# novifinancial/librabft_simulator

Measured on NVIDIA H100. Metric: simulated consensus rounds/sec (whole box), higher is better.
Workload: dtype int64

## Files before the change

__graft_entry__.py:

```python
import os
import sys

ROOT = os.path.dirname(os.path.abspath(__file__))
if ROOT not in sys.path:
    sys.path.insert(0, ROOT)


def build():
    from librabft_simulator_b200 import _build
    _build.build_product(verbose_ptxas=False)
    _build.build_oracle()
    _build.build_hostcore()
    _build.build_sweep_hostcore()
    _build.build_ct_hostcore()
    _build.build_latency_hostcore()
    _build.build_fault_hostcore()
    _build.build_block_latency_hostcore()
    _build.build_block_threshold_probe()
    import librabft_simulator_b200
    from librabft_simulator_b200 import _lib
    _lib.load()


def smoke():
    import numpy as np
    from librabft_simulator_b200 import BatchSimulator, RandomDelay, Simulator
    from tests.support import Oracle
    contexts = Simulator.new(52, 3, RandomDelay.new(10.0, 4.0), None).loop_until(1000)
    assert [c.num_commits() for c in contexts] == [27, 27, 27]
    assert [c.last_committed_state() for c in contexts] == [11134312813757838303] * 3
    seeds = np.arange(1, 65, dtype=np.uint64)
    res = BatchSimulator(seeds, 4, RandomDelay.new(10.0, 4.0)).loop_until(1000)
    ref = Oracle().run(seeds, 4, 1000)
    assert (res.commit_counts == ref.commit_counts).all()
    assert (res.last_committed_states == ref.last_states).all()
    assert (res.counters[:, :8] == ref.counters[:, :8]).all()
    print("smoke ok: 64x4 instances bit-exact vs oracle; rounds/instance = %.1f" % res.active_rounds.mean())


if __name__ == "__main__":
    build()
    print("build ok")
```

librabft_simulator_b200/_build.py:

```python
import os
import shutil
import subprocess

ROOT = os.path.dirname(os.path.dirname(os.path.abspath(__file__)))
CSRC = os.path.join(ROOT, "librabft_simulator_b200", "csrc")
LIB_PATH = os.environ.get("LBFT_LIB_PATH") or os.path.join(CSRC, "liblbft_b200.so")
ORACLE_DIR = os.path.join(ROOT, "oracle")
ORACLE_PATH = os.path.join(ORACLE_DIR, "liblbft_oracle.so")
HOSTCORE_DIR = os.path.join(ROOT, "tests", "hostcore")
HOSTCORE_PATH = os.path.join(HOSTCORE_DIR, "libhostcore.so")
SWEEP_HOSTCORE_PATH = os.path.join(HOSTCORE_DIR, "libhostcore_sweep.so")
CT_HOSTCORE_PATH = os.path.join(HOSTCORE_DIR, "libhostcore_ct.so")
LATENCY_HOSTCORE_PATH = os.path.join(HOSTCORE_DIR, "libhostcore_latency.so")
FAULT_HOSTCORE_PATH = os.path.join(HOSTCORE_DIR, "libhostcore_fault.so")
BLOCK_LATENCY_HOSTCORE_PATH = os.path.join(HOSTCORE_DIR, "libhostcore_block_latency.so")
GPUPROBE_DIR = os.path.join(ROOT, "tests", "gpuprobe")
BLOCK_THRESHOLD_PROBE_PATH = os.path.join(GPUPROBE_DIR, "libblock_threshold_probe.so")

GENCODE = ["-gencode", "arch=compute_90a,code=sm_90a"]
NVCC_FLAGS = GENCODE + ["-lineinfo", "-O3", "-std=c++17", "-Xcompiler", "-fPIC"]
PRODUCT_UNITS = ["lbft_api.cu", "k_fixed.cu", "k_scan.cu", "k_calendar.cu", "k_heap.cu", "k_wide.cu", "k_sweep_thread.cu",
                 "k_sweep_wide.cu", "k_ct_thread.cu", "k_ct_wide.cu", "k_ct_sweep_thread.cu", "k_ct_sweep_wide.cu"]
PRODUCT_HEADERS = ["kernels.cuh", "sim_core.cuh", "sim_params.h", "host_setup.hpp"]


def _newer(target, sources):
    if not os.path.exists(target):
        return False
    t = os.path.getmtime(target)
    return all(os.path.getmtime(s) <= t for s in sources)


def _run(cmd, cwd):
    proc = subprocess.run(cmd, cwd=cwd, stdout=subprocess.PIPE, stderr=subprocess.STDOUT, text=True)
    if proc.returncode != 0:
        raise RuntimeError("build failed: %s\n%s" % (" ".join(cmd), proc.stdout))
    return proc.stdout


def nvcc_path():
    return shutil.which("nvcc") or "/usr/local/cuda/bin/nvcc"


def build_product(force=False, verbose_ptxas=False, lib_path=None):
    from concurrent.futures import ThreadPoolExecutor
    lib_path = lib_path or LIB_PATH
    headers = [os.path.join(CSRC, f) for f in PRODUCT_HEADERS] + [os.path.join(ROOT, "include", "lbft.h")]
    sources = headers + [os.path.join(CSRC, u) for u in PRODUCT_UNITS]
# ... 87 lines not shown
def build_latency_hostcore(force=False):
    srcs = [os.path.join(HOSTCORE_DIR, f) for f in ("latency_hostcore.cpp", "ct_hostcore.cpp")] + [
        os.path.join(ROOT, "include", "lbft.h")] + [os.path.join(CSRC, f) for f in ("sim_core.cuh", "sim_params.h", "host_setup.hpp")] + [
        os.path.join(ORACLE_DIR, f) for f in ("oracle_capi.cpp", "lbft_oracle.hpp")]
    if not force and _newer(LATENCY_HOSTCORE_PATH, srcs):
        return LATENCY_HOSTCORE_PATH
    _run(["g++", "-O2", "-std=c++17", "-fPIC", "-shared", "-ffp-contract=off", "-Wno-unknown-pragmas", "-DLBFT_CHECK_C1",
          "-o", LATENCY_HOSTCORE_PATH, "latency_hostcore.cpp"], HOSTCORE_DIR)
    return LATENCY_HOSTCORE_PATH


def build_fault_hostcore(force=False):
    srcs = [os.path.join(HOSTCORE_DIR, f) for f in ("fault_hostcore.cpp", "ct_hostcore.cpp")] + [
        os.path.join(ROOT, "include", "lbft.h")] + [os.path.join(CSRC, f) for f in ("sim_core.cuh", "sim_params.h", "host_setup.hpp")] + [
        os.path.join(ORACLE_DIR, f) for f in ("oracle_capi.cpp", "lbft_oracle.hpp")]
    if not force and _newer(FAULT_HOSTCORE_PATH, srcs):
        return FAULT_HOSTCORE_PATH
    _run(["g++", "-O2", "-std=c++17", "-fPIC", "-shared", "-ffp-contract=off", "-Wno-unknown-pragmas", "-DLBFT_CHECK_C1",
          "-o", FAULT_HOSTCORE_PATH, "fault_hostcore.cpp"], HOSTCORE_DIR)
    return FAULT_HOSTCORE_PATH


def build_block_latency_hostcore(force=False):
    srcs = [os.path.join(HOSTCORE_DIR, f) for f in ("block_latency_hostcore.cpp", "fault_hostcore.cpp", "ct_hostcore.cpp")] + [
        os.path.join(ROOT, "include", "lbft.h")] + [os.path.join(CSRC, f) for f in ("sim_core.cuh", "sim_params.h", "host_setup.hpp")] + [
        os.path.join(ORACLE_DIR, f) for f in ("oracle_capi.cpp", "lbft_oracle.hpp")]
    if not force and _newer(BLOCK_LATENCY_HOSTCORE_PATH, srcs):
        return BLOCK_LATENCY_HOSTCORE_PATH
    _run(["g++", "-O2", "-std=c++17", "-fPIC", "-shared", "-ffp-contract=off", "-Wno-unknown-pragmas", "-DLBFT_CHECK_C1",
          "-o", BLOCK_LATENCY_HOSTCORE_PATH, "block_latency_hostcore.cpp"], HOSTCORE_DIR)
    return BLOCK_LATENCY_HOSTCORE_PATH


def build_block_threshold_probe(force=False):
    srcs = [os.path.join(GPUPROBE_DIR, "block_threshold_probe.cu")] + [os.path.join(CSRC, f) for f in ("sim_core.cuh", "sim_params.h")]
    if not force and _newer(BLOCK_THRESHOLD_PROBE_PATH, srcs):
        return BLOCK_THRESHOLD_PROBE_PATH
    _run([nvcc_path()] + NVCC_FLAGS + ["-shared", "-o", BLOCK_THRESHOLD_PROBE_PATH, "block_threshold_probe.cu"], GPUPROBE_DIR)
    return BLOCK_THRESHOLD_PROBE_PATH


def build_all(force=False):
    return (build_product(force), build_oracle(force), build_hostcore(force), build_sweep_hostcore(force), build_ct_hostcore(force),
            build_latency_hostcore(force), build_fault_hostcore(force), build_block_latency_hostcore(force),
            build_block_threshold_probe(force))
```

librabft_simulator_b200/csrc/kernels.cuh:

```cuda
#pragma once
#include <cuda_runtime.h>

#include "host_setup.hpp"
#include "sim_core.cuh"

namespace lbft {

LBFT_LAYOUT_FN uint32_t calendar_kmask_words(const Layout& L) { return (L.cal_times + 7) / 8; }

template <int QMODE>
struct LaunchShape {
  static constexpr int kThreads = QMODE == 2 ? 32 * 4 : 32;
  static constexpr int kBlocksPerSm = QMODE == 2 ? 4 : 16;
};

template <int NMAX, int QMODE, int FX, bool REC, bool RES, bool EP, bool TDS, int TILE, bool SW, bool CT = false>
__device__ __forceinline__ void event_loop_body(const Params& P, double* s_zx, double* s_zf, double* s_thr, uint32_t* s_queue,
                                                const uint32_t* set_of, const SweepSet* sets, int32_t* times = nullptr,
                                                bool faults = false) {
  static_assert(TILE == 32 || ((QMODE == 3 || QMODE == 2) && !REC && !RES && !EP && !TDS), "sparse tiles: plain kernels over the calendar / shared-memory queue");
  for (int i = threadIdx.x; i < 257; i += blockDim.x) {
    s_zx[i] = P.zig_x[i];
    s_zf[i] = P.zig_f[i];
  }
  const bool thr_fits = !SW && P.delay_kmax != 0 && P.delay_kmax + 2 <= kThrSmem;
  if (thr_fits)
    for (uint32_t i = threadIdx.x; i < P.delay_kmax + 2; i += blockDim.x) s_thr[i] = P.delay_thr[i];
  __syncthreads();
  const uint32_t gthread = blockIdx.x * blockDim.x + threadIdx.x;
  const uint32_t tile = gthread >> 5, lane = gthread & 31;
  const uint32_t inst = tile * TILE + lane;
  if (lane >= TILE || inst >= P.num_instances) return;
  const uint32_t total_words = FX ? fixed_layout(FX).total_words : P.L.total_words;
  TileMem<TILE> mem{P.state + (size_t)tile * total_words * TILE, lane};
  uint32_t* sk = nullptr;
  uint16_t* sd = nullptr;
  if (QMODE == 2) {
    const uint32_t warp = threadIdx.x >> 5, qcap = P.L.queue_cap;
    uint32_t* base = s_queue + (size_t)warp * (qcap * 32 + qcap * 16);
    sk = base + lane;
    sd = reinterpret_cast<uint16_t*>(base + qcap * 32) + lane;
  }
  constexpr bool KS = QMODE == 3 && TILE < 32;
  Core<TileMem<TILE>, NMAX, QMODE, FX, REC, RES, 1, EP, TDS, KS, SW, CT> core(P, mem, s_zx, s_zf, thr_fits ? s_thr : P.delay_thr, sk, sd);
  if (KS) core.km = s_queue + (size_t)(threadIdx.x >> 5) * calendar_kmask_words(FX ? fixed_layout(FX) : P.L) * TILE + lane;
  if constexpr (CT) core.ct = times + (size_t)inst * (core.L.num_nodes + 1) * core.L.round_cap;
  if constexpr (SW) {
    core.bind_set(faults ? &reinterpret_cast<const SweepSetFaults*>(sets)[set_of[inst]].set : sets + set_of[inst]);
    core.bind_faults(faults);
  }
  if (RES && (P.run_flags & 1u)) core.restore_regs();
  else core.init(P.seeds[inst]);
  core.run();
  core.finalize(inst);
  if (RES) core.save_regs();
}

template <int NMAX, int QMODE, int FX = FX_NONE, bool REC = false, bool RES = false, bool EP = false, bool TDS = false, int TILE = 32>
__global__ void __launch_bounds__(LaunchShape<QMODE>::kThreads, LaunchShape<QMODE>::kBlocksPerSm) lbft_event_loop_kernel(const __grid_constant__ Params P) {
  __shared__ double s_zx[257];
  __shared__ double s_zf[257];
  __shared__ double s_thr[kThrSmem];
  extern __shared__ uint32_t s_queue[];
  event_loop_body<NMAX, QMODE, FX, REC, RES, EP, TDS, TILE, false>(P, s_zx, s_zf, s_thr, s_queue, nullptr, nullptr);
}

template <int NMAX, int QMODE, int TILE = 32>
__global__ void __launch_bounds__(LaunchShape<QMODE>::kThreads, LaunchShape<QMODE>::kBlocksPerSm) lbft_sweep_event_loop_kernel(const __grid_constant__ SweepParams S) {
  __shared__ double s_zx[257];
  __shared__ double s_zf[257];
  extern __shared__ uint32_t s_queue[];
  event_loop_body<NMAX, QMODE, FX_NONE, false, false, false, false, TILE, true>(S.P, s_zx, s_zf, nullptr, s_queue, S.set_of, S.sets, nullptr,
                                                                               S.faults != 0);
}

LBFT_LAYOUT_FN int wide_warps(int g) { return g == 32 ? 1 : 4; }
LBFT_LAYOUT_FN int wide_blocks_per_sm(int g) { return 16 / wide_warps(g); }
// ... 204 lines not shown
```

librabft_simulator_b200/csrc/sim_core.cuh:

```cuda
#pragma once
#include <stddef.h>
#include <stdint.h>

#include <type_traits>

#include "sim_params.h"

#if defined(__CUDACC__)
#define LBFT_HD __host__ __device__ __forceinline__
#define LBFT_COLD inline __host__ __device__ __noinline__
#else
#define LBFT_HD inline
#define LBFT_COLD inline __attribute__((noinline))
#include <cmath>
#endif

namespace lbft {

enum : uint32_t {
  ST_DONE = 1u << 0,
  ST_ROUND_OVERFLOW = 1u << 1,
  ST_QUEUE_OVERFLOW = 1u << 2,
  ST_PAYLOAD_OVERFLOW = 1u << 3,
  ST_INVARIANT = 1u << 4,
// ... 63 lines not shown
  double d;
  __builtin_memcpy(&d, &b, 8);
  return d;
#endif
}
LBFT_HD uint64_t rotl64(uint64_t x, int k) { return (x << k) | (x >> (64 - k)); }
LBFT_HD void st_evict_first(int32_t* p, int32_t v) {
#if defined(__CUDA_ARCH__)
  __stcs(p, v);
#else
  *p = v;
#endif
}

struct SipWords {
  uint64_t v0, v1, v2, v3, nbytes;
  LBFT_HD SipWords() : v0(0x736f6d6570736575ULL), v1(0x646f72616e646f6dULL), v2(0x6c7967656e657261ULL), v3(0x7465646279746573ULL), nbytes(0) {}
  LBFT_HD void round() {
    v0 += v1; v1 = rotl64(v1, 13); v1 ^= v0; v0 = rotl64(v0, 32);
    v2 += v3; v3 = rotl64(v3, 16); v3 ^= v2;
    v0 += v3; v3 = rotl64(v3, 21); v3 ^= v0;
    v2 += v1; v1 = rotl64(v1, 17); v1 ^= v2; v2 = rotl64(v2, 32);
  }
  LBFT_HD void write_u64(uint64_t m) { v3 ^= m; round(); v0 ^= m; nbytes += 8; }
  LBFT_HD uint64_t finish() {
    uint64_t b = nbytes << 56;
    v3 ^= b; round(); v0 ^= b;
    v2 ^= 0xff;
    round(); round(); round();
    return v0 ^ v1 ^ v2 ^ v3;
  }
};

template <int STRIDE_>
struct TileMem {
  static constexpr int STRIDE = STRIDE_;
  uint32_t* tile;
  uint32_t lane;
  LBFT_HD uint32_t* at(uint32_t w) const { return tile + (size_t)w * STRIDE + lane; }
  LBFT_HD uint32_t ld(uint32_t w) const { return tile[(size_t)w * STRIDE + lane]; }
  LBFT_HD void st(uint32_t w, uint32_t v) const { tile[(size_t)w * STRIDE + lane] = v; }
  LBFT_HD uint64_t* at64(uint32_t wbase) const { return reinterpret_cast<uint64_t*>(tile + (size_t)wbase * STRIDE + lane * 2); }
};

template <int NMAX>
struct AuthorList;
template <>
struct AuthorList<16> {
  uint64_t v = 0;
  uint32_t len = 0;
  LBFT_HD void clear() { v = 0; len = 0; }
  LBFT_HD void push(uint32_t a) { v |= (uint64_t)a << (4 * len); len++; }
  LBFT_HD uint32_t get(uint32_t i) const { return (uint32_t)(v >> (4 * i)) & 15u; }
  LBFT_HD void swap(uint32_t i, uint32_t j) {
    uint64_t d = ((v >> (4 * i)) ^ (v >> (4 * j))) & 15u;
    v ^= (d << (4 * i)) | (d << (4 * j));
  }
  LBFT_HD void fill_others(uint32_t n_nodes, uint32_t self) {
    const uint64_t iota = 0xfedcba9876543210ULL;
    uint64_t lowmask = self ? ((1ULL << (4 * self)) - 1) : 0;
    v = (iota & lowmask) | ((iota >> 4) & ~lowmask);
    len = n_nodes - 1;
    if (len < 16) v &= (1ULL << (4 * len)) - 1;
  }
};
template <>
struct AuthorList<64> {
  uint8_t a[64];
  uint32_t len = 0;
  LBFT_HD void clear() { len = 0; }
  LBFT_HD void push(uint32_t x) { a[len++] = (uint8_t)x; }
  LBFT_HD uint32_t get(uint32_t i) const { return a[i]; }
  LBFT_HD void swap(uint32_t i, uint32_t j) { uint8_t t = a[i]; a[i] = a[j]; a[j] = t; }
  LBFT_HD void fill_others(uint32_t n_nodes, uint32_t self) {
    len = 0;
// ... 315 lines not shown
  LBFT_HD void clear(const Mem& m, const Layout& L, uint32_t wl, uint32_t* km_) {
    km = km_; cur = 0; pool_free = PAY_NONE; pool_next = 0;
    for (uint32_t w = wl; w < (L.cal_times + 7) / 8; w += G) km_st(m, L, w, 0);
  }
  template <class V>
  LBFT_HD void walk_regs(V& v) { v(cur); v(pool_free); v(pool_next); }
};

template <int QMODE, class Mem, int G, bool KS>
using QueueFor = typename std::conditional<QMODE == 0, HeapQueue<Mem, G>, typename std::conditional<QMODE == 1, HbmScanQueue<Mem, G>,
    typename std::conditional<QMODE == 2, SmemScanQueue<Mem, G>, CalendarQueue<Mem, G, KS>>::type>::type>::type;

template <class Mem, int NMAX, int QMODE, int FX = 0, bool REC = false, bool RES = false, int G = 1, bool EP = false,
          bool TDS = false, bool KS = false, bool SW = false, bool CT = false>
struct Core {
  static_assert(!KS || (QMODE == 3 && !RES && G == 1), "shared-memory occupancy words: calendar queue, one-shot thread kernels");
  static_assert(!SW || (FX == FX_NONE && !REC && !RES && !EP && !TDS), "sweeps: plain single-epoch generic kernels only");
  static_assert(!CT || (!REC && !RES && !EP && !TDS), "commit times: one-shot single-epoch runs");
  static constexpr bool FIXED = FX != FX_NONE;
  static constexpr bool MAY_SILENT = FX == FX_NONE || FX == FX_COMMITTEE64;
  static_assert(!(FIXED && EP), "the compile-time layout is single-epoch");
  static_assert(!(TDS && (FIXED || REC || RES || EP || G > 1)), "true data-sync: plain single-epoch thread kernels only");
  static_assert(!(FIXED && (REC || RES)), "the compile-time layout has neither a round-switch table nor a save area");
  static_assert(G == 1 || G == 8 || G == 16 || G == 32, "one thread, or a group of 8 / 16 / 32 lanes per instance");
  static_assert(G == 1 || !(REC || RES), "the wide kernel has no recording / resumable variants");
  static constexpr bool PACK = FX == FX_DEFAULT4;
  static_assert(!PACK || (NMAX <= 16 && G == 1), "compact encoding: the four-author thread kernel");
  static constexpr bool WIDE = G > 1;
  uint32_t wl = 0;
  uint32_t gm = 0xffffffffu;
  WideScratch* ws = nullptr;
  static constexpr bool ELIDE = !(REC || RES);
  static constexpr int S = Mem::STRIDE;
  const Params& P;
  const Layout L;
  Mem m;
  const double* zx;
  const double* zf;
  const double* thr;
  const SweepSet* sw = nullptr;
  bool faults = false;
  using Queue = QueueFor<QMODE, Mem, G, KS>;
  Queue q;
  uint32_t* km = nullptr;
  int32_t* ct = nullptr;
  uint64_t s0, s1, s2, s3;
  uint32_t draws;
  uint32_t stamp;
  uint32_t qsize;
  uint32_t status;
  int32_t clock;
  uint32_t pay_free, pay_next;
  uint32_t proc0, proc1, proc2, proc3, cancelled, max_queue, sched_notify, dedup;
  uint32_t win;
  int32_t part_until;
  uint64_t part_open;
  uint32_t rs_pend;
  uint32_t cc0, cc1, cc2, cc3;

  LBFT_HD Core(const Params& p, Mem mem, const double* zx_, const double* zf_, const double* thr_, uint32_t* sk = nullptr,
               uint16_t* sd = nullptr)
      : P(p), L(FIXED ? fixed_layout(FX) : p.L), m(mem), zx(zx_), zf(zf_), thr(thr_) { q.attach(sk, sd); }

  LBFT_HD void bind_set(const SweepSet* set) {
    sw = set;
    thr = P.delay_thr + set->thr_off;
// ... 103 lines not shown
    uint32_t word, shift, mask;
  };
  LBFT_HD static constexpr PackedField packed_field(uint32_t f) {
    switch (f) {
      case F_STARTUP: return {0, 0, ~0u};
      case F_IGNORE: return {1, 0, ~0u};
      case F_PM_START: return {2, 0, ~0u};
      case F_PM_DUR: return {3, 0, ~0u};
      case F_PM_PERIOD: return {4, 0, ~0u};
      case F_LQA: return {5, 0, ~0u};
      case F_TRK_TIME: return {6, 0, ~0u};
      case F_LAST_TIMER: return {7, 0, ~0u};
      case F_BALLOT: return {8, 0, ~0u};
      case F_TOW: return {9, 0, ~0u};
      case F_CUR: return {10, 0, 0xffu};
      case F_HQC: return {10, 8, 0xffu};
      case F_HTC: return {10, 16, 0xffu};
      case F_HCR: return {10, 24, 0xffu};
      case F_HCC: return {11, 0, 0xffu};
      case F_LVR: return {11, 8, 0xffu};
      case F_LOCKED: return {11, 16, 0xffu};
      case F_PMR: return {11, 24, 0xffu};
      case F_TRK_HCR: return {12, 0, 0xffu};
      case F_LC_ROUND: return {12, 8, 0xffu};
      case F_TC_ROUND: return {12, 16, 0xffu};
      case F_COMMITS: return {12, 24, 0xffu};
      case F_FLAGS: return {13, 0, 0xff0fu};
      case F_NSCALAR + 2: return {13, 4, 0xfu};
      case F_NSCALAR: return {13, 16, 0xfu};
      case F_NSCALAR + 1: return {13, 20, 0xfu};
      default: return {13, 24, 0xffu};
    }
  }
  LBFT_HD uint32_t node_ld(uint32_t b, uint32_t f) const {
    if constexpr (PACK) {
      const PackedField pf = packed_field(f);
      return (m.ld(b + pf.word) >> pf.shift) & pf.mask;
    }
    return m.ld(b + f);
  }
  LBFT_HD void node_st(uint32_t b, uint32_t f, uint32_t v) const {
    if constexpr (PACK) {
      const PackedField pf = packed_field(f);
      m.st(b + pf.word, (m.ld(b + pf.word) & ~(pf.mask << pf.shift)) | ((v & pf.mask) << pf.shift));
    } else {
      m.st(b + f, v);
    }
  }
  using mask_t = typename std::conditional<(NMAX > 32), uint64_t, uint32_t>::type;
  LBFT_HD static mask_t ld_mask(const uint32_t* p) {
    uint64_t v = p[0];
    if (NMAX > 32) v |= (uint64_t)p[S] << 32;
    return (mask_t)v;
  }
  LBFT_HD static void st_mask(uint32_t* p, mask_t v) {
    p[0] = (uint32_t)v;
    if (NMAX > 32) p[S] = (uint32_t)((uint64_t)v >> 32);
  }
  LBFT_HD static uint32_t ld_u16(const uint32_t* p, uint32_t i) { return (p[(i >> 1) * S] >> (16 * (i & 1))) & 0xffffu; }
  LBFT_HD static void st_u16(uint32_t* p, uint32_t i, uint32_t v) {
    reinterpret_cast<uint16_t*>(p + (i >> 1) * S)[i & 1] = (uint16_t)v;
  }
  LBFT_HD bool mbit_test(uint32_t w, uint32_t r) const { return (m.ld(w + (r >> 5)) >> (r & 31)) & 1u; }
  LBFT_HD void mbit_set(uint32_t w, uint32_t r) const { m.st(w + (r >> 5), m.ld(w + (r >> 5)) | (1u << (r & 31))); }
  LBFT_HD uint32_t chain_prev(uint32_t g) const {
    uint32_t e = (g & 2) ? ((g & 1) ? cc3 : cc2) : ((g & 1) ? cc1 : cc0);
    if ((e >> 16) == g) return e & 0xffffu;
    return m.ld(L.chain_base + 2 * g) & 0xffffu;
  }
  LBFT_HD static constexpr bool multi() { return EP; }
  LBFT_HD uint32_t chain_parent(uint32_t g) const {
    const uint32_t p = chain_prev(g);
    if (!multi()) return p;
    const uint32_t e = g / L.rspan;
    return p ? e * L.rspan + p : m.ld(L.einit_base + e);
  }
  LBFT_HD void chain_cache_put(uint32_t r, uint32_t prev) {
    uint32_t e = (r << 16) | prev;
    if ((r & 3) == 0) cc0 = e;
    if ((r & 3) == 1) cc1 = e;
    if ((r & 3) == 2) cc2 = e;
    if ((r & 3) == 3) cc3 = e;
  }

  struct NodeRegs {
    uint32_t f[F_NSCALAR];
    mask_t vmask, tmask, tcmask;
    uint32_t cw;
    uint32_t chb, chq, cpd;
    uint32_t dirty;
    uint32_t gb;
    uint32_t* nb;
  };
  LBFT_HD static uint32_t epoch_of(const NodeRegs& d) { return (d.f[F_FLAGS] >> FL_EPOCH_SHIFT) & FL_EPOCH_BITS; }
  LBFT_HD void load_node(uint32_t n, NodeRegs& d) {
    uint32_t* nb = m.at(nbase(n));
    d.nb = nb;
    if constexpr (PACK) {
      uint32_t w[kPackedScalarWords];
#pragma unroll
      for (int i = 0; i < (int)kPackedScalarWords; i++) w[i] = nb[i * S];
      auto get = [&](uint32_t f) { const PackedField pf = packed_field(f); return (w[pf.word] >> pf.shift) & pf.mask; };
#pragma unroll
      for (int i = 0; i < (int)F_NSCALAR; i++) d.f[i] = get(i);
      d.vmask = get(F_NSCALAR);
      d.tmask = get(F_NSCALAR + 1);
      d.tcmask = get(F_NSCALAR + 2);
    } else {
#pragma unroll
      for (int i = 0; i < (int)F_NSCALAR; i++) d.f[i] = nb[i * S];
      d.vmask = ld_mask(nb + L.n_vmask * S);
      d.tmask = ld_mask(nb + L.n_tmask * S);
      d.tcmask = ld_mask(nb + L.n_tcmask * S);
    }
    d.chb = nb[(L.n_hasblk + win) * S];
    d.chq = nb[(L.n_hasqc + win) * S];
    d.cpd = nb[(L.n_pend + win) * S];
    d.gb = multi() ? epoch_of(d) * L.rspan : 0u;
    uint32_t want = (d.gb + d.f[F_CUR]) >> 5;
    if (want != win) {
      d.chb = nb[(L.n_hasblk + want) * S];
      d.chq = nb[(L.n_hasqc + want) * S];
      d.cpd = nb[(L.n_pend + want) * S];
      win = want;
    }
    d.cw = want;
    d.dirty = 0;
  }
  LBFT_HD void store_node(const NodeRegs& d) const {
    uint32_t* nb = d.nb;
    if constexpr (PACK) {
      uint32_t w[kPackedScalarWords] = {};
      auto put = [&](uint32_t f, uint32_t v) { const PackedField pf = packed_field(f); w[pf.word] |= (v & pf.mask) << pf.shift; };
#pragma unroll
      for (int i = 0; i < (int)F_NSCALAR; i++) put(i, d.f[i]);
      put(F_NSCALAR, d.vmask);
      put(F_NSCALAR + 1, d.tmask);
      put(F_NSCALAR + 2, d.tcmask);
#pragma unroll
      for (int i = 0; i < (int)kPackedScalarWords; i++) nb[i * S] = w[i];
    } else {
#pragma unroll
      for (int i = 0; i < (int)F_NSCALAR; i++) nb[i * S] = d.f[i];
      st_mask(nb + L.n_vmask * S, d.vmask);
      st_mask(nb + L.n_tmask * S, d.tmask);
      st_mask(nb + L.n_tcmask * S, d.tcmask);
    }
    if (d.dirty & 1) nb[(L.n_hasblk + d.cw) * S] = d.chb;
    if (d.dirty & 2) nb[(L.n_hasqc + d.cw) * S] = d.chq;
    if (d.dirty & 4) nb[(L.n_pend + d.cw) * S] = d.cpd;
  }
  LBFT_HD uint32_t bword(const NodeRegs& d, uint32_t base, uint32_t cached, uint32_t r) const {
    return (r >> 5) == d.cw ? cached : d.nb[(base + (r >> 5)) * S];
  }
  LBFT_HD bool has_blk(const NodeRegs& d, uint32_t r) const { r += d.gb; return (bword(d, L.n_hasblk, d.chb, r) >> (r & 31)) & 1u; }
  LBFT_HD bool has_qc(const NodeRegs& d, uint32_t r) const { r += d.gb; return (bword(d, L.n_hasqc, d.chq, r) >> (r & 31)) & 1u; }
  LBFT_HD bool is_pend(const NodeRegs& d, uint32_t r) const { r += d.gb; return (bword(d, L.n_pend, d.cpd, r) >> (r & 31)) & 1u; }
  LBFT_HD void bput(NodeRegs& d, uint32_t base, uint32_t& cached, uint32_t dirty_bit, uint32_t r, bool on) const {
    uint32_t bit = 1u << (r & 31);
    if ((r >> 5) == d.cw) {
      cached = on ? (cached | bit) : (cached & ~bit);
      d.dirty |= dirty_bit;
    } else {
      uint32_t* p = d.nb + (base + (r >> 5)) * S;
      *p = on ? (*p | bit) : (*p & ~bit);
    }
  }
  LBFT_HD void put_timeout_hcbr(const NodeRegs& d, uint32_t a, uint32_t hcbr) const {
    if constexpr (PACK) reinterpret_cast<uint8_t*>(d.nb + kPackedTimeoutHcbr * S)[a] = (uint8_t)hcbr;
    else st_u16(d.nb + L.n_thcbr * S, a, hcbr);
  }
  LBFT_HD void copy_timeout_hcbr_to_tc(const NodeRegs& d) const {
    if constexpr (PACK) {
      d.nb[kPackedTcHcbr * S] = d.nb[kPackedTimeoutHcbr * S];
    } else {
      group_sync<G>(gm);
      for (uint32_t i = wl; i < L.hcbr_words; i += G) d.nb[(L.n_tchcbr + i) * S] = d.nb[(L.n_thcbr + i) * S];
      group_sync<G>(gm);
    }
  }
  LBFT_HD void set_blk(NodeRegs& d, uint32_t r) const { bput(d, L.n_hasblk, d.chb, 1u, d.gb + r, true); }
  LBFT_HD void set_qc(NodeRegs& d, uint32_t r) const { bput(d, L.n_hasqc, d.chq, 2u, d.gb + r, true); }
  LBFT_HD void set_pend(NodeRegs& d, uint32_t r, bool on) const { bput(d, L.n_pend, d.cpd, 4u, d.gb + r, on); }

  LBFT_HD static uint32_t election(const NodeRegs& d) { return (d.f[F_FLAGS] & FL_ELECTION_MASK) >> FL_ELECTION_SHIFT; }
  LBFT_HD static void set_election(NodeRegs& d, uint32_t e) { d.f[F_FLAGS] = (d.f[F_FLAGS] & ~FL_ELECTION_MASK) | (e << FL_ELECTION_SHIFT); }
  LBFT_HD static uint32_t leader_of(const NodeRegs& d) { return (d.f[F_FLAGS] >> FL_LEADER_SHIFT) & 0xffu; }

  LBFT_HD bool push_event(int32_t time, uint32_t kind, uint32_t data) {
    uint32_t st = stamp++;
    if (stamp >= Queue::kStampLimit) status |= ST_QUEUE_OVERFLOW;
    if (time > P.max_clock) return false;
    if (qsize >= L.queue_cap) { status |= ST_QUEUE_OVERFLOW; return false; }
    q.put(m, L, qsize, time, kind, st, data);
    qsize++;
    if (qsize > max_queue) max_queue = qsize;
    return true;
  }
  LBFT_HD void pop_event(int32_t& time, uint32_t& kind, uint32_t& data) {
    q.take(m, L, qsize, wl, gm, time, kind, data);
    qsize--;
  }

  static constexpr uint32_t kPayRef = PACK ? 1 : 2;
  LBFT_HD uint32_t pay_word(uint32_t s) const { return L.pay_base + s * (PACK ? 4u : L.pay_words); }
  LBFT_HD uint32_t* pay_at(uint32_t s) const { return m.at(pay_word(s)); }
  LBFT_HD uint32_t pay_refs(uint32_t s) const { return m.ld(pay_word(s) + kPayRef); }
  LBFT_HD const uint32_t* pay_hcbr(const uint32_t* pb, int which) const { return pb + (PACK ? 2u + which : (which ? L.p_curhcbr : L.p_tchcbr)) * S; }
  LBFT_HD static uint32_t hcbr_of(const uint32_t* hp, uint32_t a) {
    if constexpr (PACK) return (hp[0] >> (8 * a)) & 0xffu;
    else return ld_u16(hp, a);
  }
  LBFT_HD uint32_t pay_alloc() {
    uint32_t s;
    if (L.payload_cap <= 32) {
      if (pay_free == 0) { status |= ST_PAYLOAD_OVERFLOW; return PAY_NONE; }
      s = ctz32(pay_free);
      pay_free &= pay_free - 1;
      if (s >= pay_next) pay_next = s + 1;
      return s;
    }
    if (pay_free != PAY_NONE) {
      s = pay_free;
      pay_free = pay_refs(s) & 0xffffu;
    } else if (pay_next < L.payload_cap) {
      s = pay_next++;
    } else {
      status |= ST_PAYLOAD_OVERFLOW;
      s = PAY_NONE;
    }
    return s;
  }
  LBFT_HD void pay_release(uint32_t s) {
    if (L.payload_cap <= 32) { pay_free |= 1u << s; return; }
    m.st(pay_word(s) + kPayRef, pay_free);
    pay_free = s;
  }
  LBFT_HD void pay_unref(uint32_t slot, uint32_t w2) {
    uint32_t refs = (w2 & 0xffffu) - 1;
    if (refs == 0) pay_release(slot);
    else m.st(pay_word(slot) + kPayRef, (w2 & 0xffff0000u) | refs);
  }

  LBFT_HD void update_current_round(NodeRegs& d, uint32_t round) {
    if (round <= d.f[F_CUR]) return;
    if (round >= L.rspan) { status |= ST_ROUND_OVERFLOW; return; }
    d.f[F_CUR] = round;
    d.f[F_FLAGS] &= ~(FL_PROPOSED | FL_ELECTION_MASK);
    d.tmask = 0;
    d.vmask = 0;
    d.f[F_TOW] = 0;
    d.f[F_BALLOT] = 0;
  }
  LBFT_HD bool state_available(const NodeRegs& d, uint32_t prev) const {
    if (multi()) {
      if (prev == 0) return d.f[F_LC_ROUND] == m.ld(L.einit_base + epoch_of(d));
      return d.f[F_LC_ROUND] == d.gb + prev || is_pend(d, prev);
    }
    if (d.f[F_LC_ROUND] == prev) return true;
    if (prev == 0) return false;
    return is_pend(d, prev);
  }
  LBFT_HD void insert_block(NodeRegs& d, uint32_t r) {
    if (has_blk(d, r)) return;
    uint32_t prev = chain_prev(d.gb + r);
    if (prev != 0 && !has_qc(d, prev)) return;
    if (r == d.f[F_CUR]) d.f[F_FLAGS] |= FL_PROPOSED;
    set_blk(d, r);
  }
  LBFT_HD void insert_vote(NodeRegs& d, uint32_t r, uint32_t author) {
    if (r != d.f[F_CUR]) return;
    if (!has_blk(d, r)) return;
    if ((d.vmask >> author) & 1) return;
    d.vmask |= (mask_t)1 << author;
// ... 191 lines not shown
        a.next = clk;
      }
    }
    process_commits(d, n);
    bool trk_new_epoch = false;
    if (multi()) {
      const uint32_t e = epoch_of(d), te = (d.f[F_FLAGS] >> FL_TRK_EPOCH_SHIFT) & FL_EPOCH_BITS;
      if (e > te) {
        trk_new_epoch = true;
        d.f[F_FLAGS] = (d.f[F_FLAGS] & ~(FL_EPOCH_BITS << FL_TRK_EPOCH_SHIFT)) | (e << FL_TRK_EPOCH_SHIFT);
      }
    }
    if (trk_new_epoch || d.f[F_HCR] > d.f[F_TRK_HCR]) {
      d.f[F_TRK_HCR] = d.f[F_HCR];
      d.f[F_TRK_TIME] = (uint32_t)clk;
    }
    int32_t tl = (int32_t)d.f[F_TRK_TIME] > (int32_t)d.f[F_LQA] ? (int32_t)d.f[F_TRK_TIME] : (int32_t)d.f[F_LQA];
    int32_t deadline = tl + tci();
    if (clk >= deadline) {
      a.query_all = true;
      deadline = clk + tci();
    }
    if (deadline < a.next) a.next = deadline;
    if (a.query_all) d.f[F_LQA] = (uint32_t)clk;
    return a;
  }

  struct HcbrRegs {
    uint32_t tc[2], cur[2];
  };
  LBFT_HD void prefetch_hcbr(const NodeRegs& d, HcbrRegs& h) const {
    const bool has_tc = d.f[F_FLAGS] & FL_HAS_TC;
    if constexpr (PACK) {
      h.tc[0] = has_tc ? d.nb[kPackedTcHcbr * S] : 0u;
      h.cur[0] = d.tmask ? d.nb[kPackedTimeoutHcbr * S] : 0u;
      return;
    }
    if (L.hcbr_words > 2) return;
#pragma unroll
    for (uint32_t i = 0; i < 2; i++) {
      h.tc[i] = (has_tc && i < L.hcbr_words) ? d.nb[(L.n_tchcbr + i) * S] : 0u;
      h.cur[i] = (d.tmask && i < L.hcbr_words) ? d.nb[(L.n_thcbr + i) * S] : 0u;
    }
  }
  LBFT_HD void write_notification(uint32_t n, const NodeRegs& d, uint32_t slot, uint32_t refs, const HcbrRegs& h) {
    uint32_t* pb = pay_at(slot);
    bool has_tc = d.f[F_FLAGS] & FL_HAS_TC;
    uint32_t vote = (uint32_t)((d.vmask >> n) & 1);
    uint32_t prop = (d.f[F_CUR] == d.f[F_PMR] && (d.f[F_FLAGS] & FL_PROPOSED) && leader_of(d) == n) ? 1u : 0u;
    uint32_t ep = 0;
    if (multi()) {
      ep = epoch_of(d);
      if (((d.f[F_FLAGS] >> FL_PM_EPOCH_SHIFT) & FL_EPOCH_BITS) != ep) prop = 0;
    }
    if constexpr (PACK) {
      pb[0] = d.f[F_HCC] | (d.f[F_HQC] << 8) | (d.f[F_CUR] << 16) | ((has_tc ? d.f[F_TC_ROUND] : 0u) << 24);
      pb[kPayRef * S] = refs | ((vote | (prop << 1)) << 16) | ((has_tc ? d.tcmask : 0u) << 24) | (d.tmask << 28);
      if (has_tc) pb[2 * S] = h.tc[0];
      if (d.tmask) pb[3 * S] = h.cur[0];
      return;
    }
    pb[0] = d.f[F_HCC] | (d.f[F_HQC] << 16);
    pb[1 * S] = d.f[F_CUR] | ((has_tc ? d.f[F_TC_ROUND] : 0u) << 16);
    pb[2 * S] = refs | ((vote | (prop << 1)) << 16) | (ep << 18);
    st_mask(pb + L.p_tcmask * S, has_tc ? d.tcmask : (mask_t)0);
    st_mask(pb + L.p_curmask * S, d.tmask);
    if (L.hcbr_words <= 2) {
#pragma unroll
      for (uint32_t i = 0; i < 2; i++) {
        if (has_tc && i < L.hcbr_words) pb[(L.p_tchcbr + i) * S] = h.tc[i];
        if (d.tmask && i < L.hcbr_words) pb[(L.p_curhcbr + i) * S] = h.cur[i];
      }
    } else {
      if (has_tc)
        for (uint32_t i = wl; i < L.hcbr_words; i += G) pb[(L.p_tchcbr + i) * S] = d.nb[(L.n_tchcbr + i) * S];
      if (d.tmask)
        for (uint32_t i = wl; i < L.hcbr_words; i += G) pb[(L.p_curhcbr + i) * S] = d.nb[(L.n_thcbr + i) * S];
      group_sync<G>(gm);
    }
  }
  LBFT_HD bool handle_notification(NodeRegs& d, uint32_t slot, uint32_t sender) {
    uint32_t* pb = pay_at(slot);
    uint32_t hcc, hqc, cur_s, tc_round, w2;
    mask_t tcm, curm;
    if constexpr (PACK) {
      const uint32_t w0 = pb[0];
      w2 = pb[kPayRef * S];
      hcc = w0 & 0xffu, hqc = (w0 >> 8) & 0xffu, cur_s = (w0 >> 16) & 0xffu, tc_round = w0 >> 24;
      tcm = (w2 >> 24) & 0xfu, curm = w2 >> 28;
    } else {
      const uint32_t w0 = pb[0], w1 = pb[1 * S];
      w2 = pb[2 * S];
      tcm = ld_mask(pb + L.p_tcmask * S), curm = ld_mask(pb + L.p_curmask * S);
      hcc = w0 & 0xffffu, hqc = w0 >> 16, cur_s = w1 & 0xffffu, tc_round = w1 >> 16;
    }
    bool vote = (w2 >> 16) & 1, prop = (w2 >> 17) & 1;
    bool should_sync = false;
    if (multi()) {
      const uint32_t se = (w2 >> 18) & FL_EPOCH_BITS, e = epoch_of(d);
      if (se != e) {
        pay_unref(slot, w2);
        return se > e;
      }
    }
#pragma unroll 1
    for (int which = 0; which < 2; which++) {
      uint32_t q = which ? hqc : hcc;
      if (q) {
        insert_qc(d, q);
        should_sync |= which ? (q > d.f[F_HQC]) : (q > d.f[F_HCR] + 2);
      }
    }
    if (prop) insert_block(d, cur_s);
    insert_timeout_groups(d, pb, tc_round, cur_s, tcm, curm);
    if (vote) insert_vote(d, cur_s, sender);
    pay_unref(slot, w2);
    return should_sync;
  }
  LBFT_HD void insert_timeout_groups(NodeRegs& d, const uint32_t* pb, uint32_t tc_round, uint32_t cur_s, mask_t tcm, mask_t curm) {
#pragma unroll 1
// ... 95 lines not shown
    return push_event(t, kind, receiver | (sender << 8) | (slot << 16));
  }
  template <bool W = WIDE>
  LBFT_HD typename std::enable_if<W, AuthorListShared>::type make_list() const { return AuthorListShared(ws->list); }
  template <bool W = WIDE>
  LBFT_HD typename std::enable_if<!W, AuthorList<(NMAX <= 16 ? 16 : 64)>>::type make_list() const { return AuthorList<(NMAX <= 16 ? 16 : 64)>(); }
  LBFT_HD void push_timer(uint32_t n, NodeRegs& d, int32_t t) {
    if (ELIDE && (uint32_t)t == d.f[F_LAST_TIMER]) {
      stamp++;
      if (t <= P.max_clock) { proc3++; cancelled++; dedup++; }
      return;
    }
    d.f[F_LAST_TIMER] = (uint32_t)t;
    push_event(t, EV_TIMER, n | (n << 8) | (PAY_NONE << 16));
  }

  LBFT_HD void init(uint64_t seed) {
    const uint32_t N = L.num_nodes;
    seed_rng(seed, s0, s1, s2, s3);
    draws = 0; stamp = 0; qsize = 0; status = 0; clock = 0;
    pay_free = L.payload_cap <= 32 ? (L.payload_cap == 32 ? 0xffffffffu : ((1u << L.payload_cap) - 1)) : PAY_NONE;
    pay_next = 0;
    proc0 = proc1 = proc2 = proc3 = cancelled = max_queue = sched_notify = dedup = 0;
    win = 0;
    cc0 = cc1 = cc2 = cc3 = 0;
    part_until = 0; part_open = 0;
    if (REC) {
      rs_pend = 0;
      for (uint32_t w = 0; w < N * (L.round_cap + 1); w++) m.st(rs_table_base(L) + w, 0);
    }
    q.clear(m, L, wl, km);
    if constexpr (PACK) {
      for (uint32_t n = 0; n < N; n++) {
        for (uint32_t w = 0; w < kPackedWords; w++) m.st(nbase(n) + w, 0);
        for (uint32_t w = L.n_hasblk; w < L.node_words; w++) m.st(nbase(n) + w, 0);
      }
    } else {
      for (uint32_t w = wl; w < N * L.node_words; w += G) m.st(L.node_base + w, 0);
    }
    for (uint32_t w = wl; w < 2 * L.rset_words; w += G) m.st(L.created_base + w, 0);
    if (multi())
      for (uint32_t w = wl; w < L.epochs; w += G) m.st(L.einit_base + w, 0);
    group_sync<G>(gm);
    if (L.part_windows) {
      uint64_t k0 = s0, k1 = s1, k2 = s2, k3 = s3;
      uint32_t kd = draws;
      seed_rng(seed ^ 0xD1B54A32D192ED03ULL, s0, s1, s2, s3);
      uint64_t nsub = N >= 64 ? 0xfffffffffffffffeULL : ((1ULL << N) - 2);
      for (uint32_t k = 0; k < part_windows(); k++) {
        int64_t t0 = (int64_t)gen_range_u64((uint64_t)P.max_clock + 1);
        int64_t len = 1 + (int64_t)gen_range_u64(part_max_len() ? part_max_len() : 1);
        uint64_t mask = N >= 2 ? 1 + gen_range_u64(nsub) : 0;
        m.st(L.part_base + 4 * k, (uint32_t)t0);
        m.st(L.part_base + 4 * k + 1, (uint32_t)(t0 + len));
        m.st(L.part_base + 4 * k + 2, (uint32_t)mask);
        m.st(L.part_base + 4 * k + 3, (uint32_t)(mask >> 32));
      }
      if constexpr (SW)
        for (uint32_t k = part_windows(); k < L.part_windows; k++)
          for (uint32_t w = 0; w < 4; w++) m.st(L.part_base + 4 * k + w, 0);
      s0 = k0; s1 = k1; s2 = k2; s3 = k3;
      draws = kd;
    }
#pragma unroll 1
    for (uint32_t n = 0; n < N; n++) {
      int32_t startup = sample_delay() + 1;
      uint32_t b = nbase(n);
// ... 347 lines not shown
```

Measured before the change: 204.3 million.

## Store packed node words and payload slots as per-lane contiguous blocks

Adds a lane-block layout option to TileMem that is enabled for the FX_DEFAULT4 fixed layout. In that layout each lane's packed node words and 4-word payload slots sit next to each other in memory instead of being strided across the tile. Node and payload loads and stores become 16-byte vector accesses (uint4/uint2), which cuts the number of memory instructions per node load, store and notification. The trade-off is that a warp's accesses are no longer coalesced across lanes. The change also adds a host-core build for verification.

Measured after the change: 221.9 million, median of 6. 1.09x the previous value.

```diff
diff --git a/__graft_entry__.py b/__graft_entry__.py
--- a/__graft_entry__.py
+++ b/__graft_entry__.py
@@ -16,6 +16,7 @@
     _build.build_latency_hostcore()
     _build.build_fault_hostcore()
     _build.build_block_latency_hostcore()
+    _build.build_lane_block_hostcore()
     _build.build_block_threshold_probe()
     import librabft_simulator_b200
     from librabft_simulator_b200 import _lib
diff --git a/librabft_simulator_b200/_build.py b/librabft_simulator_b200/_build.py
--- a/librabft_simulator_b200/_build.py
+++ b/librabft_simulator_b200/_build.py
@@ -14,6 +14,7 @@
 LATENCY_HOSTCORE_PATH = os.path.join(HOSTCORE_DIR, "libhostcore_latency.so")
 FAULT_HOSTCORE_PATH = os.path.join(HOSTCORE_DIR, "libhostcore_fault.so")
 BLOCK_LATENCY_HOSTCORE_PATH = os.path.join(HOSTCORE_DIR, "libhostcore_block_latency.so")
+LANE_BLOCK_HOSTCORE_PATH = os.path.join(HOSTCORE_DIR, "libhostcore_lane_block.so")
 GPUPROBE_DIR = os.path.join(ROOT, "tests", "gpuprobe")
 BLOCK_THRESHOLD_PROBE_PATH = os.path.join(GPUPROBE_DIR, "libblock_threshold_probe.so")
 
@@ -167,6 +168,16 @@
     return BLOCK_LATENCY_HOSTCORE_PATH
 
 
+def build_lane_block_hostcore(force=False):
+    srcs = [os.path.join(HOSTCORE_DIR, "lane_block_hostcore.cpp")] + [
+        os.path.join(CSRC, f) for f in ("sim_core.cuh", "sim_params.h", "host_setup.hpp")]
+    if not force and _newer(LANE_BLOCK_HOSTCORE_PATH, srcs):
+        return LANE_BLOCK_HOSTCORE_PATH
+    _run(["g++", "-O2", "-std=c++17", "-fPIC", "-shared", "-ffp-contract=off", "-Wno-unknown-pragmas", "-DLBFT_CHECK_C1",
+          "-o", LANE_BLOCK_HOSTCORE_PATH, "lane_block_hostcore.cpp"], HOSTCORE_DIR)
+    return LANE_BLOCK_HOSTCORE_PATH
+
+
 def build_block_threshold_probe(force=False):
     srcs = [os.path.join(GPUPROBE_DIR, "block_threshold_probe.cu")] + [os.path.join(CSRC, f) for f in ("sim_core.cuh", "sim_params.h")]
     if not force and _newer(BLOCK_THRESHOLD_PROBE_PATH, srcs):
@@ -178,4 +189,4 @@
 def build_all(force=False):
     return (build_product(force), build_oracle(force), build_hostcore(force), build_sweep_hostcore(force), build_ct_hostcore(force),
             build_latency_hostcore(force), build_fault_hostcore(force), build_block_latency_hostcore(force),
-            build_block_threshold_probe(force))
+            build_lane_block_hostcore(force), build_block_threshold_probe(force))
diff --git a/librabft_simulator_b200/csrc/kernels.cuh b/librabft_simulator_b200/csrc/kernels.cuh
--- a/librabft_simulator_b200/csrc/kernels.cuh
+++ b/librabft_simulator_b200/csrc/kernels.cuh
@@ -32,7 +32,8 @@
   const uint32_t inst = tile * TILE + lane;
   if (lane >= TILE || inst >= P.num_instances) return;
   const uint32_t total_words = FX ? fixed_layout(FX).total_words : P.L.total_words;
-  TileMem<TILE> mem{P.state + (size_t)tile * total_words * TILE, lane};
+  using Mem = TileMem<TILE, FX == FX_DEFAULT4>;
+  Mem mem{P.state + (size_t)tile * total_words * TILE, lane};
   uint32_t* sk = nullptr;
   uint16_t* sd = nullptr;
   if (QMODE == 2) {
@@ -42,7 +43,7 @@
     sd = reinterpret_cast<uint16_t*>(base + qcap * 32) + lane;
   }
   constexpr bool KS = QMODE == 3 && TILE < 32;
-  Core<TileMem<TILE>, NMAX, QMODE, FX, REC, RES, 1, EP, TDS, KS, SW, CT> core(P, mem, s_zx, s_zf, thr_fits ? s_thr : P.delay_thr, sk, sd);
+  Core<Mem, NMAX, QMODE, FX, REC, RES, 1, EP, TDS, KS, SW, CT> core(P, mem, s_zx, s_zf, thr_fits ? s_thr : P.delay_thr, sk, sd);
   if (KS) core.km = s_queue + (size_t)(threadIdx.x >> 5) * calendar_kmask_words(FX ? fixed_layout(FX) : P.L) * TILE + lane;
   if constexpr (CT) core.ct = times + (size_t)inst * (core.L.num_nodes + 1) * core.L.round_cap;
   if constexpr (SW) {
diff --git a/librabft_simulator_b200/csrc/sim_core.cuh b/librabft_simulator_b200/csrc/sim_core.cuh
--- a/librabft_simulator_b200/csrc/sim_core.cuh
+++ b/librabft_simulator_b200/csrc/sim_core.cuh
@@ -119,15 +119,21 @@
   }
 };
 
-template <int STRIDE_>
+template <int STRIDE_, bool LB_ = false>
 struct TileMem {
   static constexpr int STRIDE = STRIDE_;
+  static constexpr bool LB = LB_;
+  static constexpr int BLOCK_PITCH = LB ? 1 : STRIDE;
   uint32_t* tile;
   uint32_t lane;
   LBFT_HD uint32_t* at(uint32_t w) const { return tile + (size_t)w * STRIDE + lane; }
   LBFT_HD uint32_t ld(uint32_t w) const { return tile[(size_t)w * STRIDE + lane]; }
   LBFT_HD void st(uint32_t w, uint32_t v) const { tile[(size_t)w * STRIDE + lane] = v; }
   LBFT_HD uint64_t* at64(uint32_t wbase) const { return reinterpret_cast<uint64_t*>(tile + (size_t)wbase * STRIDE + lane * 2); }
+  LBFT_HD static constexpr size_t block_word(uint32_t base, uint32_t K, uint32_t k, uint32_t lane) {
+    return LB ? (size_t)base * STRIDE + lane * K + k : ((size_t)base + k) * STRIDE + lane;
+  }
+  LBFT_HD uint32_t* block(uint32_t base, uint32_t K) const { return tile + block_word(base, K, 0, lane); }
 };
 
 template <int NMAX>
@@ -509,6 +515,8 @@
   WideScratch* ws = nullptr;
   static constexpr bool ELIDE = !(REC || RES);
   static constexpr int S = Mem::STRIDE;
+  static_assert(!Mem::LB || PACK, "lane blocks: the compact node words and slots only");
+  static constexpr int PS = Mem::BLOCK_PITCH;
   const Params& P;
   const Layout L;
   Mem m;
@@ -678,17 +686,49 @@
       default: return {13, 24, 0xffu};
     }
   }
+  LBFT_HD uint32_t* pk_at(uint32_t b) const { return m.block(b, kPackedWords); }
+  template <int K>
+  LBFT_HD static void ld_block(const uint32_t* p, uint32_t (&w)[K]) {
+    static_assert(K % 4 == 0, "whole 16-byte units");
+#if defined(__CUDA_ARCH__)
+    if constexpr (Mem::LB) {
+#pragma unroll
+      for (int i = 0; i < K / 4; i++) {
+        const uint4 v = reinterpret_cast<const uint4*>(p)[i];
+        w[4 * i] = v.x, w[4 * i + 1] = v.y, w[4 * i + 2] = v.z, w[4 * i + 3] = v.w;
+      }
+      return;
+    }
+#endif
+#pragma unroll
+    for (int i = 0; i < K; i++) w[i] = p[i * PS];
+  }
+  template <int K>
+  LBFT_HD static void st_block(uint32_t* p, const uint32_t (&w)[K]) {
+    static_assert(K % 4 == 0 || K % 4 == 2, "whole 8-byte units");
+#if defined(__CUDA_ARCH__)
+    if constexpr (Mem::LB) {
+#pragma unroll
+      for (int i = 0; i < K / 4; i++) reinterpret_cast<uint4*>(p)[i] = make_uint4(w[4 * i], w[4 * i + 1], w[4 * i + 2], w[4 * i + 3]);
+      if constexpr (K % 4 != 0) reinterpret_cast<uint2*>(p)[K / 2 - 1] = make_uint2(w[K - 2], w[K - 1]);
+      return;
+    }
+#endif
+#pragma unroll
+    for (int i = 0; i < K; i++) p[i * PS] = w[i];
+  }
   LBFT_HD uint32_t node_ld(uint32_t b, uint32_t f) const {
     if constexpr (PACK) {
       const PackedField pf = packed_field(f);
-      return (m.ld(b + pf.word) >> pf.shift) & pf.mask;
+      return (pk_at(b)[pf.word * PS] >> pf.shift) & pf.mask;
     }
     return m.ld(b + f);
   }
   LBFT_HD void node_st(uint32_t b, uint32_t f, uint32_t v) const {
     if constexpr (PACK) {
       const PackedField pf = packed_field(f);
-      m.st(b + pf.word, (m.ld(b + pf.word) & ~(pf.mask << pf.shift)) | ((v & pf.mask) << pf.shift));
+      uint32_t* p = pk_at(b) + pf.word * PS;
+      *p = (*p & ~(pf.mask << pf.shift)) | ((v & pf.mask) << pf.shift);
     } else {
       m.st(b + f, v);
     }
@@ -737,15 +777,16 @@
     uint32_t dirty;
     uint32_t gb;
     uint32_t* nb;
+    uint32_t* pk;
   };
   LBFT_HD static uint32_t epoch_of(const NodeRegs& d) { return (d.f[F_FLAGS] >> FL_EPOCH_SHIFT) & FL_EPOCH_BITS; }
   LBFT_HD void load_node(uint32_t n, NodeRegs& d) {
     uint32_t* nb = m.at(nbase(n));
     d.nb = nb;
     if constexpr (PACK) {
-      uint32_t w[kPackedScalarWords];
-#pragma unroll
-      for (int i = 0; i < (int)kPackedScalarWords; i++) w[i] = nb[i * S];
+      d.pk = pk_at(nbase(n));
+      uint32_t w[kPackedWords];
+      ld_block(d.pk, w);
       auto get = [&](uint32_t f) { const PackedField pf = packed_field(f); return (w[pf.word] >> pf.shift) & pf.mask; };
 #pragma unroll
       for (int i = 0; i < (int)F_NSCALAR; i++) d.f[i] = get(i);
@@ -783,8 +824,7 @@
       put(F_NSCALAR, d.vmask);
       put(F_NSCALAR + 1, d.tmask);
       put(F_NSCALAR + 2, d.tcmask);
-#pragma unroll
-      for (int i = 0; i < (int)kPackedScalarWords; i++) nb[i * S] = w[i];
+      st_block(d.pk, w);
     } else {
 #pragma unroll
       for (int i = 0; i < (int)F_NSCALAR; i++) nb[i * S] = d.f[i];
@@ -813,12 +853,12 @@
     }
   }
   LBFT_HD void put_timeout_hcbr(const NodeRegs& d, uint32_t a, uint32_t hcbr) const {
-    if constexpr (PACK) reinterpret_cast<uint8_t*>(d.nb + kPackedTimeoutHcbr * S)[a] = (uint8_t)hcbr;
+    if constexpr (PACK) reinterpret_cast<uint8_t*>(d.pk + kPackedTimeoutHcbr * PS)[a] = (uint8_t)hcbr;
     else st_u16(d.nb + L.n_thcbr * S, a, hcbr);
   }
   LBFT_HD void copy_timeout_hcbr_to_tc(const NodeRegs& d) const {
     if constexpr (PACK) {
-      d.nb[kPackedTcHcbr * S] = d.nb[kPackedTimeoutHcbr * S];
+      d.pk[kPackedTcHcbr * PS] = d.pk[kPackedTimeoutHcbr * PS];
     } else {
       group_sync<G>(gm);
       for (uint32_t i = wl; i < L.hcbr_words; i += G) d.nb[(L.n_tchcbr + i) * S] = d.nb[(L.n_thcbr + i) * S];
@@ -850,9 +890,12 @@
 
   static constexpr uint32_t kPayRef = PACK ? 1 : 2;
   LBFT_HD uint32_t pay_word(uint32_t s) const { return L.pay_base + s * (PACK ? 4u : L.pay_words); }
-  LBFT_HD uint32_t* pay_at(uint32_t s) const { return m.at(pay_word(s)); }
-  LBFT_HD uint32_t pay_refs(uint32_t s) const { return m.ld(pay_word(s) + kPayRef); }
-  LBFT_HD const uint32_t* pay_hcbr(const uint32_t* pb, int which) const { return pb + (PACK ? 2u + which : (which ? L.p_curhcbr : L.p_tchcbr)) * S; }
+  LBFT_HD uint32_t* pay_at(uint32_t s) const { return PACK ? m.block(pay_word(s), 4) : m.at(pay_word(s)); }
+  LBFT_HD uint32_t* pay_ref_at(uint32_t s) const { return PACK ? pay_at(s) + kPayRef * PS : m.at(pay_word(s) + kPayRef); }
+  LBFT_HD uint32_t pay_refs(uint32_t s) const { return *pay_ref_at(s); }
+  LBFT_HD const uint32_t* pay_hcbr(const uint32_t* pb, int which) const {
+    return PACK ? pb + (2u + which) * PS : pb + (which ? L.p_curhcbr : L.p_tchcbr) * S;
+  }
   LBFT_HD static uint32_t hcbr_of(const uint32_t* hp, uint32_t a) {
     if constexpr (PACK) return (hp[0] >> (8 * a)) & 0xffu;
     else return ld_u16(hp, a);
@@ -879,13 +922,13 @@
   }
   LBFT_HD void pay_release(uint32_t s) {
     if (L.payload_cap <= 32) { pay_free |= 1u << s; return; }
-    m.st(pay_word(s) + kPayRef, pay_free);
+    *pay_ref_at(s) = pay_free;
     pay_free = s;
   }
   LBFT_HD void pay_unref(uint32_t slot, uint32_t w2) {
     uint32_t refs = (w2 & 0xffffu) - 1;
     if (refs == 0) pay_release(slot);
-    else m.st(pay_word(slot) + kPayRef, (w2 & 0xffff0000u) | refs);
+    else *pay_ref_at(slot) = (w2 & 0xffff0000u) | refs;
   }
 
   LBFT_HD void update_current_round(NodeRegs& d, uint32_t round) {
@@ -1143,8 +1186,8 @@
   LBFT_HD void prefetch_hcbr(const NodeRegs& d, HcbrRegs& h) const {
     const bool has_tc = d.f[F_FLAGS] & FL_HAS_TC;
     if constexpr (PACK) {
-      h.tc[0] = has_tc ? d.nb[kPackedTcHcbr * S] : 0u;
-      h.cur[0] = d.tmask ? d.nb[kPackedTimeoutHcbr * S] : 0u;
+      h.tc[0] = has_tc ? d.pk[kPackedTcHcbr * PS] : 0u;
+      h.cur[0] = d.tmask ? d.pk[kPackedTimeoutHcbr * PS] : 0u;
       return;
     }
     if (L.hcbr_words > 2) return;
@@ -1165,10 +1208,10 @@
       if (((d.f[F_FLAGS] >> FL_PM_EPOCH_SHIFT) & FL_EPOCH_BITS) != ep) prop = 0;
     }
     if constexpr (PACK) {
-      pb[0] = d.f[F_HCC] | (d.f[F_HQC] << 8) | (d.f[F_CUR] << 16) | ((has_tc ? d.f[F_TC_ROUND] : 0u) << 24);
-      pb[kPayRef * S] = refs | ((vote | (prop << 1)) << 16) | ((has_tc ? d.tcmask : 0u) << 24) | (d.tmask << 28);
-      if (has_tc) pb[2 * S] = h.tc[0];
-      if (d.tmask) pb[3 * S] = h.cur[0];
+      const uint32_t w[4] = {d.f[F_HCC] | (d.f[F_HQC] << 8) | (d.f[F_CUR] << 16) | ((has_tc ? d.f[F_TC_ROUND] : 0u) << 24),
+                             refs | ((vote | (prop << 1)) << 16) | ((has_tc ? d.tcmask : 0u) << 24) | (d.tmask << 28), h.tc[0],
+                             h.cur[0]};
+      st_block(pb, w);
       return;
     }
     pb[0] = d.f[F_HCC] | (d.f[F_HQC] << 16);
@@ -1195,8 +1238,10 @@
     uint32_t hcc, hqc, cur_s, tc_round, w2;
     mask_t tcm, curm;
     if constexpr (PACK) {
-      const uint32_t w0 = pb[0];
-      w2 = pb[kPayRef * S];
+      uint32_t w[4];
+      ld_block(pb, w);
+      const uint32_t w0 = w[0];
+      w2 = w[kPayRef];
       hcc = w0 & 0xffu, hqc = (w0 >> 8) & 0xffu, cur_s = (w0 >> 16) & 0xffu, tc_round = w0 >> 24;
       tcm = (w2 >> 24) & 0xfu, curm = w2 >> 28;
     } else {
@@ -1358,7 +1403,8 @@
     q.clear(m, L, wl, km);
     if constexpr (PACK) {
       for (uint32_t n = 0; n < N; n++) {
-        for (uint32_t w = 0; w < kPackedWords; w++) m.st(nbase(n) + w, 0);
+        const uint32_t zero[kPackedWords] = {};
+        st_block(pk_at(nbase(n)), zero);
         for (uint32_t w = L.n_hasblk; w < L.node_words; w++) m.st(nbase(n) + w, 0);
       }
     } else {
```
